# privefl/bigsnpr

Measured on AMD Instinct MI355X. Metric: SNP-cols/sec for bed_randomSVD k=20 (m*passes/wall), higher is better.
Workload: dtype i8 (2-bit codes x 24-bit (early block steps) / 16-bit (late block steps) fixed-point image of the fp64 basis in int8 slices, exact int32 MFMA accumulation; fp64 panel algebra and Rayleigh-Ritz)

## Files before the change

bigsnpr_amd/csrc/api.hip:

```cpp
#include <cxxabi.h>

#include <algorithm>
#include <cmath>
#include <cstring>
#include <limits>
#include <memory>

#include "bsn_internal.hpp"

namespace bsn {

static std::vector<int32_t> to_i32(const int64_t *ind, int64_t len, int64_t limit, const char *what) {
  std::vector<int32_t> v((size_t)len);
  if (!ind) {
    if (len > limit)
      fail("Tested %lld < %lld. Subscript out of bounds (%s).", (long long)(len - 1), (long long)limit, what);
    for (int64_t i = 0; i < len; i++) v[(size_t)i] = (int32_t)i;
    return v;
  }
  for (int64_t i = 0; i < len; i++) {
    if (ind[i] < 0 || ind[i] >= limit)
      fail("Tested %lld < %lld. Subscript out of bounds (%s).", (long long)ind[i], (long long)limit,
           what);
    v[(size_t)i] = (int32_t)ind[i];
// ... 318 lines not shown
  const double deno = deno_x * deno_y - num * num;
  res[j + (int64_t)k * m] = (deno == 0 || nona < 2) ? __longlong_as_double(0x7ff8000000000000LL)
                                                    : num * sqrt((nona - 2) / deno);
}
#pragma clang fp contract(on)

}

using namespace bsn;

extern "C" {

int bsn_selftest(void) {
  return guarded([&] {
    require_gpu();
    selftest();
  });
}

int bsn_op_last_kernel(bsn_op *op, char *buf, int64_t len) {
  return guarded([&] {
    if (!buf || len < 1) fail("bsn_op_last_kernel: no buffer");
    buf[0] = 0;
    if (!op->last_kernel) return;
    const char *mangled = hipKernelNameRefByPtr(op->last_kernel, op->bed->stream);
    if (!mangled) return;
    int status = 1;
    char *dem = abi::__cxa_demangle(mangled, nullptr, nullptr, &status);
    std::string name = (status == 0 && dem) ? dem : mangled;
    free(dem);
    const size_t par = name.find('(');
    if (par != std::string::npos) name.resize(par);
    snprintf(buf, (size_t)len, "%s", name.c_str());
  });
}

int bsn_op_create(bsn_bed *bed, const int64_t *ind_row, int64_t n, const int64_t *ind_col,
                  int64_t m, const double *center, const double *scale, bsn_op **out) {
  return guarded([&] {
    std::unique_ptr<bsn_op> op(new bsn_op());
    fill_op(op.get(), bed, ind_row, n, ind_col, m, center, scale);
    *out = op.release();
  });
}

int bsn_op_destroy(bsn_op *op) {
  return guarded([&] {
    if (op) {
      (void)hipSetDevice(op->bed->device);
      delete op;
    }
  });
}

int bsn_op_set_slices(bsn_op *op, int slices) {
  return guarded([&] {
    if (slices < 1 || slices > 7) fail("slices must be in 1..7");
    op->slices = slices;
  });
}

int bsn_op_prod(bsn_op *op, const double *d_X, int64_t ldx, int nvec, double *d_Y, int64_t ldy) {
  return guarded([&] {
    BSN_HIP(hipSetDevice(op->bed->device));
    op_prod(op, d_X, ldx, nvec, d_Y, ldy);
  });
// ... 455 lines not shown
```

bigsnpr_amd/csrc/bsn_internal.hpp:

```cpp
#pragma once
#include <hip/hip_runtime.h>
#include <stdint.h>

#include <atomic>
#include <cstdarg>
#include <cstdio>
#include <functional>
#include <cstdlib>
#include <memory>
#include <stdexcept>
#include <string>
#include <vector>

#include "bigsnpr_hip.h"

namespace bsn {
inline const char *abl_getenv(const char *name) {
#ifdef BSN_ABLATION
  return getenv(name);
#else
  (void)name;
  return nullptr;
#endif
}
// ... 319 lines not shown
void slab_upload_range(bsn_bed *b, int64_t j0, int64_t cnt);
struct SlabPart {
  bsn_bed *img;
  const std::vector<int64_t> &P;
  const std::vector<int64_t> &local;
  int64_t count() const { return (int64_t)P.size(); }
  const double *gather(const double *src, std::vector<double> &buf) const;
  void place(void *out, const void *part, size_t col_bytes) const;
};
void slab_walk(bsn_bed *bed, const int64_t *ind_col, int64_t m, const std::function<void(const SlabPart &)> &f);

hipEvent_t comm_time_begin(bsn_comm *c, hipStream_t st);
void comm_time_end(bsn_comm *c, hipEvent_t begin, int cls, hipStream_t st);
void comm_time_collect(bsn_comm *c, double ms[kCommClasses], int count[kCommClasses]);
bool comm_abort(bsn_comm *c);
void comm_allreduce_sum(bsn_comm *c, double *d_buf, int64_t count, hipStream_t st);
void comm_reduce_scatter_sum(bsn_comm *c, const double *d_send, double *d_recv, int64_t recv_count,
                             hipStream_t st);
void comm_all_gather(bsn_comm *c, const double *d_send, double *d_recv, int64_t send_count, hipStream_t st);

void op_poll_stats(bsn_op *op);
void op_na_blocks(bsn_op *op, int digit_cols);
void op_prod(bsn_op *op, const double *d_X, int64_t ldx, int nvec, double *d_Y, int64_t ldy);
void op_prod_acc(bsn_op *op, const double *d_X, int64_t ldx, int nvec, double *d_Y, int64_t ldy, double beta);
struct ProdSegment {
  int bs = 0, off = 0;
  const int32_t *d_rows = nullptr;
  double *d_out = nullptr;
};
bool op_prod_segments(bsn_op *op, const double *d_X, int64_t ldx, int nvec, int pieces, int stride, int nseg,
                      const ProdSegment *segs, const std::function<void(int)> &after);
void op_cprod(bsn_op *op, const double *d_X, int64_t ldx, int nvec, double *d_Z, int64_t ldz);
void op_cprod_prequant(bsn_op *op, const double *d_X, int64_t ldx, int nvec);
void op_cprod_raw(bsn_op *op, const double *d_X, int64_t ldx, int nvec, double *d_P, double *d_Q,
                  int64_t ld);
void require_bits(const bsn_bed *b, int bits, const char *what);
void op_row_sums_sq(bsn_op *op, double *d_out);
void op_row_counts(bsn_op *op, double *d_out);
void counts_weighted(bsn_op *op, const double *d_w, int64_t n_sub, int32_t *d_counts);
void counts_grouped(bsn_op *op, const int32_t *d_rows, const int32_t *d_group, int64_t n, int32_t G, const int32_t *d_gsize,
                    bool one_digit, int32_t *d_table, double ms_out[3]);
void group_counts_device(bsn_bed *bed, const int64_t *ind_row, int64_t n, const int32_t *group, int32_t G,
                         const int64_t *ind_col, int64_t m, DevBuf<int32_t> &d_table, double ms_out[3]);
void selftest();
void roctx_push(const char *name);
void roctx_pop();
struct RoctxRange {
  explicit RoctxRange(const char *name) { roctx_push(name); }
  ~RoctxRange() { roctx_pop(); }
  RoctxRange(const RoctxRange &) = delete;
  RoctxRange &operator=(const RoctxRange &) = delete;
};
void require_resident(const bsn_bed *b, const char *what);
void prof_begin(bsn_op *op, int kind, bool more = false);
void prof_end(bsn_op *op);
void prof_collect(bsn_op *op, double ms[kProfKinds], int count[kProfKinds]);

}
```

bigsnpr_amd/csrc/matvec.hip:

```cpp
#include <cmath>
#include <cstdlib>

#include "bsn_internal.hpp"
#include "byte_plan.hpp"
#include "prod_plan.hpp"
#include "prodt_sparse.hpp"
#include <type_traits>

namespace bsn {

typedef int v4i __attribute__((ext_vector_type(4)));
typedef int v8i __attribute__((ext_vector_type(8)));

static thread_local const void *g_last_kernel = nullptr;
#define BSN_KLAUNCH(kern, ...)                 \
  do {                                         \
    g_last_kernel = (const void *)(kern);      \
    hipLaunchKernelGGL(kern, __VA_ARGS__);     \
  } while (0)

__device__ __forceinline__ uint32_t lut4(uint32_t lut, uint32_t sel) {
  return __builtin_amdgcn_perm(lut, lut, sel);
}
__device__ __forceinline__ uint32_t perm8(uint32_t hi, uint32_t lo, uint32_t sel) {
  return __builtin_amdgcn_perm(hi, lo, sel);
}

constexpr uint32_t kLutG0 = 0x00020100u;
constexpr uint32_t kLutNA = 0x01000000u;
constexpr uint32_t kLutHom2 = 0x00010000u;
constexpr uint32_t kLutHet = 0x00000100u;
constexpr uint32_t kLutRaw = 0xFFFFFFFFu;

struct VecMeta {
// ... 166 lines not shown
        }
      }
    }
    for (int p = 0; p < nplanes; p++)
#pragma unroll
      for (int s = 0; s < S; s++) {
        const int col = v * S + s;
        int8_t *dst = q + ((kb * nplanes + p) * ncol + col) * 16;
        *(uint4 *)dst = p == 0 ? uint4{pk[0][s][0], pk[0][s][1], pk[0][s][2], pk[0][s][3]}
                               : uint4{pk[1][s][0], pk[1][s][1], pk[1][s][2], pk[1][s][3]};
      }
  }
  for (int off = 32; off > 0; off >>= 1) {
    shi += __shfl_down(shi, off); slo += __shfl_down(slo, off);
    shi2 += __shfl_down(shi2, off); slo2 += __shfl_down(slo2, off);
  }
  if (tid == 0) {
    atomicAdd((unsigned long long *)&meta[v].sum_hi, (unsigned long long)shi);
    atomicAdd((unsigned long long *)&meta[v].sum_lo, (unsigned long long)slo);
    if (mode >= 1) {
      atomicAdd((unsigned long long *)&meta[v].sum2_hi, (unsigned long long)shi2);
      atomicAdd((unsigned long long *)&meta[v].sum2_lo, (unsigned long long)slo2);
    }
  }
}

template <int NB, int NPLANE, int KC, bool RAW0, bool STATS, bool CONTIG, int TILES = 2, int WAVES = 8, int MINW = 1,
          int TAG = 0, bool TILED = false, int SGB = 0, bool NASKIP = false>
__global__ __launch_bounds__(64 * WAVES, MINW) void k_cprod(const uint8_t *__restrict__ img, int64_t pitch,
                                               const int32_t *__restrict__ cols, int64_t col0,
                                               int64_t m, const int8_t *__restrict__ xq,
                                               int32_t *__restrict__ acc_out, int64_t m_out,
                                               uint32_t lutA, uint32_t lutB, uint32_t lutC,
                                               int32_t *__restrict__ counts, int32_t n_pad_samples) {
  constexpr int NCOL = 16 * NB;
  constexpr int LD = KC / 256;
  constexpr int XS = KC / 16 * NCOL;
  __shared__ uint4 xs[2][XS];
  const int tid = threadIdx.x, wave = tid >> 6, lane = tid & 63;
  const int c = lane & 15, g = lane >> 4;
  constexpr int NT = 64 * WAVES;
  const int64_t wg_base = (int64_t)blockIdx.x * (WAVES * 16 * TILES);
  const int64_t snp_base = wg_base + wave * (16 * TILES);
  const uint8_t *rowp[TILES];
  uint32_t voff[TILES];
#pragma unroll
  for (int t = 0; t < TILES; t++) {
    int64_t j = snp_base + t * 16 + c;
    if (j > m - 1) j = m - 1;
    int64_t col = CONTIG ? col0 + j : (int64_t)cols[j];
    rowp[t] = img + col * pitch + g * 16;
    voff[t] = TILED ? (uint32_t)((((j - wg_base) >> 6) * (pitch >> 8)) * 16384 + (j & 63) * 256 + g * 16)
                    : (uint32_t)((j - wg_base) * pitch + g * 16);
  }
  static_assert(!TILED || (CONTIG && (WAVES * 16 * TILES) % 64 == 0), "streaming layout: whole 64-variant blocks");
  const __amdgpu_buffer_rsrc_t rs = __builtin_amdgcn_make_buffer_rsrc(
      (void *)(TILED ? img + (((col0 + wg_base) >> 6) * (pitch >> 8)) * 16384
                     : img + (col0 + (CONTIG ? wg_base : 0)) * pitch),
      0, 0x7fffffff, 0x00020000);
  typedef unsigned int v4u __attribute__((ext_vector_type(4)));
  auto gload = [&](const int t, const int off) -> uint4 {
    if constexpr (CONTIG) {
      const int soff = TILED ? ((off >> 8) << 14) + (off & 255) : off;
      const v4u r = __builtin_amdgcn_raw_buffer_load_b128(rs, (int)voff[t], soff, 0);
      return uint4{r.x, r.y, r.z, r.w};
    } else {
      return *(const uint4 *)(rowp[t] + off);
    }
  };
  const int nchunks = (int)(pitch * 4 / KC);
  const uint4 *xq4 = (const uint4 *)xq;

  v4i acc[TILES][NPLANE][NB];
#pragma unroll
  for (int t = 0; t < TILES; t++)
#pragma unroll
    for (int p = 0; p < NPLANE; p++)
#pragma unroll
      for (int nb = 0; nb < NB; nb++) acc[t][p][nb] = v4i{0, 0, 0, 0};
  uint32_t st_lo[TILES], st_hi[TILES], st_na[TILES];
#pragma unroll
  for (int t = 0; t < TILES; t++) st_lo[t] = st_hi[t] = st_na[t] = 0;

  constexpr int NX = (XS + NT - 1) / NT;
  static_assert(NX <= 4, "staging registers");
  constexpr bool XFULL = (XS % NT == 0);
  uint4 ga[2][TILES][LD];
  uint4 xr0 = {0, 0, 0, 0}, xr1 = {0, 0, 0, 0}, xr2 = {0, 0, 0, 0}, xr3 = {0, 0, 0, 0};
#pragma unroll
  for (int t = 0; t < TILES; t++)
#pragma unroll
    for (int it = 0; it < LD; it++) ga[0][t][it] = gload(t, it * 64);
  auto staged = [&](const int x) -> bool { return XFULL || tid + x * NT < XS; };
  if (staged(0)) xs[0][tid] = xq4[tid];
  if constexpr (NX > 1) if (staged(1)) xs[0][tid + NT] = xq4[tid + NT];
  if constexpr (NX > 2) if (staged(2)) xs[0][tid + 2 * NT] = xq4[tid + 2 * NT];
  if constexpr (NX > 3) if (staged(3)) xs[0][tid + 3 * NT] = xq4[tid + 3 * NT];
#pragma unroll
  for (int t = 0; t < TILES; t++)
#pragma unroll
    for (int it = 0; it < LD; it++)
      ga[1][t][it] = gload(t, (nchunks > 1 ? KC / 4 : 0) + it * 64);
  __syncthreads();

  auto chunk = [&](auto SETC, const int ch) {
    constexpr int SET = decltype(SETC)::value;
    const int ch1 = ch + 1 < nchunks ? ch + 1 : nchunks - 1;
    const int ch2 = ch + 2 < nchunks ? ch + 2 : nchunks - 1;
    {
      const uint4 *src = xq4 + (int64_t)ch1 * XS;
      auto at = [&](const int x) -> int { return XFULL ? tid + x * NT : (tid + x * NT < XS ? tid + x * NT : XS - 1); };
      xr0 = src[at(0)];
      if constexpr (NX > 1) xr1 = src[at(1)];
      if constexpr (NX > 2) xr2 = src[at(2)];
      if constexpr (NX > 3) xr3 = src[at(3)];
    }
    __builtin_amdgcn_sched_barrier(0);
    if constexpr (SGB & 2) __builtin_amdgcn_s_setprio(2);
    const int off2 = ch2 * (KC / 4);
    auto kstep = [&](const int t, const uint32_t w, const uint4 (&bv)[NB]) {
      uint32_t s0 = w & 0x03030303u, s1 = (w >> 2) & 0x03030303u,
               s2 = (w >> 4) & 0x03030303u, s3 = (w >> 6) & 0x03030303u;
      if constexpr (STATS) {
        const uint32_t lo = w & 0x55555555u;
        st_lo[t] += __popc(lo);
        st_hi[t] += __popc(w);
        st_na[t] += __popc(lo & (w >> 1));
      }
      static_assert(!NASKIP || (RAW0 && NPLANE == 2 && !STATS), "the skip is for the missing-value plane of the plain pass");
      bool plane1 = true;
      if constexpr (NASKIP) plane1 = __builtin_amdgcn_ballot_w64(((w & (w >> 1)) & 0x55555555u) != 0u) != 0ull;
#pragma unroll
      for (int p = 0; p < NPLANE; p++) {
        if (NASKIP && p == 1 && !plane1) continue;
        const uint32_t lut = p == 0 ? lutA : p == 1 ? lutB : lutC;
        v4i a;
        if (RAW0 && p == 0) {
          a = v4i{(int)s0, (int)s1, (int)s2, (int)s3};
        } else {
          a = v4i{(int)lut4(lut, s0), (int)lut4(lut, s1), (int)lut4(lut, s2), (int)lut4(lut, s3)};
        }
// ... 43 lines not shown
      constexpr int MSTEP = TILES * NPLANE * NB;
      __builtin_amdgcn_sched_group_barrier(0x100, NB, 0);
      __builtin_amdgcn_sched_group_barrier(0x002, 7, 0);
      auto slot = [&](auto IC) {
        constexpr int i = decltype(IC)::value;
        constexpr int nv = VSTEP * (i + 1) / MSTEP - VSTEP * i / MSTEP;
        __builtin_amdgcn_sched_group_barrier(0x008, 1, 0);
        if constexpr (nv > 0) __builtin_amdgcn_sched_group_barrier(0x002, nv, 0);
      };
      auto slots = [&](auto self, auto IC) {
        constexpr int i = decltype(IC)::value;
        if constexpr (i < MSTEP) {
          slot(IC);
          self(self, std::integral_constant<int, i + 1>{});
        }
      };
#pragma unroll
      for (int stp = 0; stp < LD * 4; stp++) {
        __builtin_amdgcn_sched_group_barrier(0x100, NB, 0);
        slots(slots, std::integral_constant<int, 0>{});
      }
      __builtin_amdgcn_sched_group_barrier(0x020, TILES * LD, 0);
    }
    __builtin_amdgcn_sched_barrier(0);
    if constexpr (SGB & 2) __builtin_amdgcn_s_setprio(0);
    {
      if (staged(0)) xs[SET ^ 1][tid] = xr0;
      if constexpr (NX > 1) if (staged(1)) xs[SET ^ 1][tid + NT] = xr1;
      if constexpr (NX > 2) if (staged(2)) xs[SET ^ 1][tid + 2 * NT] = xr2;
      if constexpr (NX > 3) if (staged(3)) xs[SET ^ 1][tid + 3 * NT] = xr3;
    }
    __syncthreads();
  };
  for (int ch = 0; ch < nchunks; ch += 2) {
    chunk(std::integral_constant<int, 0>{}, ch);
    if (ch + 1 < nchunks) chunk(std::integral_constant<int, 1>{}, ch + 1);
  }

#pragma unroll
  for (int t = 0; t < TILES; t++)
#pragma unroll
    for (int r = 0; r < 4; r++) {
      int64_t j = snp_base + t * 16 + g * 4 + r;
      if (j < m) {
#pragma unroll
        for (int p = 0; p < NPLANE; p++)
#pragma unroll
          for (int nb = 0; nb < NB; nb++)
            acc_out[((int64_t)p * m_out + j) * NCOL + nb * 16 + c] = acc[t][p][nb][r];
      }
    }
  if constexpr (STATS) {
#pragma unroll
    for (int t = 0; t < TILES; t++) {
      uint32_t lo = st_lo[t], hi = st_hi[t] - st_lo[t], na = st_na[t];
      lo += __shfl_xor(lo, 16); hi += __shfl_xor(hi, 16); na += __shfl_xor(na, 16);
      lo += __shfl_xor(lo, 32); hi += __shfl_xor(hi, 32); na += __shfl_xor(na, 32);
      const int64_t j = snp_base + t * 16 + c;
      if (g == 0 && j < m) {
        const int32_t n1 = (int32_t)(lo - na), n2 = (int32_t)(hi - na);
        *(int4 *)(counts + 4 * j) =
            int4{(int32_t)(pitch * 4) - n1 - n2 - (int32_t)na - n_pad_samples, n1, n2, (int32_t)na};
      }
    }
  }
}

__device__ __forceinline__ double horner(const int32_t *a, int S) {
  double r = 0;
  for (int s = S - 1; s >= 0; s--) r = r * 256.0 + (double)a[s];
  return r;
}
__device__ __forceinline__ double horner_sub(const int32_t *a, const int32_t *q, int k, int S) {
  double r = 0;
  for (int s = S - 1; s >= 0; s--) r = r * 256.0 + (double)((long long)a[s] - (long long)k * q[s]);
  return r;
}

template <int NCOL>
__global__ __launch_bounds__(128) void k_cprod_final(const int32_t *__restrict__ acc, int64_t m, int S, int nv,
                                                     const VecMeta *__restrict__ meta,
                                                     const double *__restrict__ center,
                                                     const double *__restrict__ scale, double *Z, int64_t ldz,
                                                     int has_q) {
  constexpr int ROW = 2 * NCOL + 1;
  __shared__ int32_t srow[128 * ROW];
  const int64_t j = (int64_t)blockIdx.x * 128 + threadIdx.x;
  if (j >= m) return;
  int32_t *my = srow + threadIdx.x * ROW;
  {
    const int4 *pa = (const int4 *)(acc + j * NCOL), *pq = (const int4 *)(acc + (m + j) * NCOL);
#pragma unroll
    for (int t = 0; t < NCOL / 4; t++) {
      const int4 x = pa[t];
      my[4 * t] = x.x; my[4 * t + 1] = x.y; my[4 * t + 2] = x.z; my[4 * t + 3] = x.w;
    }
    if (has_q) {
#pragma unroll
      for (int t = 0; t < NCOL / 4; t++) {
        const int4 x = pq[t];
        my[NCOL + 4 * t] = x.x; my[NCOL + 4 * t + 1] = x.y; my[NCOL + 4 * t + 2] = x.z; my[NCOL + 4 * t + 3] = x.w;
      }
    }
  }
  const double c = center ? center[j] : 0.0, s = scale ? scale[j] : 1.0;
  for (int v = 0; v < nv; v++) {
    const double P = has_q ? horner_sub(my + v * S, my + NCOL + v * S, 3, S) : horner(my + v * S, S);
    const double Q = has_q ? horner(my + NCOL + v * S, S) : 0.0;
    const double Sx = (double)meta[v].sum_hi * 16777216.0 + (double)meta[v].sum_lo;
    const double qs = meta[v].qscale;
    double z = qs > 0 ? (P - c * (Sx - Q)) / (s * qs) : 0.0 / s;
    if (P == 0.0 && Sx - Q == 0.0 && qs > 0) z = 0.0;
    if (meta[v].nonfinite) z = __longlong_as_double(0x7ff8000000000000LL);
    Z[j + v * ldz] = z;
  }
}

template <int NB, bool CONTIG, bool RAWP, bool HASQ = true, int TAG = 0, bool TILED = false>
__global__ __launch_bounds__(256) void k_prod(const uint8_t *__restrict__ img, int64_t pitch,
                                              const int32_t *__restrict__ cols, int64_t col0,
                                              int64_t m_pad, int64_t mc,
                                              const int8_t *__restrict__ wq,
                                              int32_t *__restrict__ acc_out, int64_t n_pad,
// ... 695 lines not shown
#pragma clang fp contract(on)

__global__ __launch_bounds__(256) void k_stats_summary(const int32_t *counts, int64_t m, int64_t n, int32_t *na,
                                                       unsigned long long *out) {
  long long s = 0, bad = 0;
  for (int64_t j = (int64_t)blockIdx.x * 256 + threadIdx.x; j < m; j += (int64_t)gridDim.x * 256) {
    const int4 c = *(const int4 *)(counts + 4 * j);
    s += c.w;
    na[j] = c.w;
    if (2 * ((int64_t)c.x + c.y + c.z) < n) bad++;
  }
  for (int off = 32; off > 0; off >>= 1) {
    s += __shfl_down(s, off);
    bad += __shfl_down(bad, off);
  }
  __shared__ long long sw[4], sb[4];
  if ((threadIdx.x & 63) == 0) {
    sw[threadIdx.x >> 6] = s;
    sb[threadIdx.x >> 6] = bad;
  }
  __syncthreads();
  if (threadIdx.x == 0) {
    s = sw[0] + sw[1] + sw[2] + sw[3];
    bad = sb[0] + sb[1] + sb[2] + sb[3];
    if (s) atomicAdd(&out[0], (unsigned long long)s);
    if (bad) atomicAdd(&out[1], (unsigned long long)bad);
  }
}

static bool use_tiled(const bsn_op *op) {
  return op->bed->d_tiled != nullptr && op->cols_contig && (op->col0 & 63) == 0;
}

template <int NPLANE, bool RAW0, bool STATS>
static void launch_cprod(bsn_op *op, int NB, const int8_t *q, int32_t *acc, uint32_t l0,
                         uint32_t l1, uint32_t l2, int32_t *counts = nullptr) {
  bsn_bed *b = op->bed;
  constexpr int KC = 512, TT = STATS ? 2 : 4;
  constexpr bool PLAIN = NPLANE == 2 && RAW0 && !STATS;
  if (b->pitch * 4 > 4000000) fail("more than 4e6 samples are not supported by the crossproduct kernel");
  const int32_t *cols = op->cols_contig ? nullptr : op->d_cols.p;
  const int32_t npad = (int32_t)(b->pitch * 4 - b->n);
  CprodFacts f;
  f.NB = NB, f.plain = PLAIN, f.stats = STATS, f.cols_contig = op->cols_contig, f.tiled = use_tiled(op);
  f.warm = op->prof_kind_override == 3, f.na_skip = op->na_skip_c;
  const CprodKernel k = choose_cprod(f);
  const uint8_t *image = k.tiled ? b->d_tiled : b->d_img;
  const int per_wg = 16 * k.tiles * k.waves;
  const dim3 grid((unsigned)((op->m + per_wg - 1) / per_wg)), block(64 * k.waves);
#define BSN_CPROD(NBV, CONTIGV, TV, WV, TAGV, TILEDV, SGBV, NASKIPV)                                                   \
  if (k == CprodKernel{NBV, CONTIGV, TV, WV, TAGV, TILEDV, SGBV, NASKIPV}) {                                           \
    BSN_KLAUNCH((k_cprod<NBV, NPLANE, KC, RAW0, STATS, CONTIGV, TV, WV, 1, TAGV, TILEDV, SGBV, NASKIPV>), grid, block, \
                0, b->stream, image, b->pitch, cols, op->col0, op->m, q, acc, op->m, l0, l1, l2, counts, npad);        \
    BSN_HIP(hipGetLastError());                                                                                        \
    return;                                                                                                            \
  }
  BSN_CPROD(1, false, 2, 8, 0, false, 0, false)
  BSN_CPROD(1, true, 2, 8, 0, false, 0, false)
  BSN_CPROD(1, true, 2, 8, 1, false, 0, false)
  BSN_CPROD(1, true, TT, 8, 0, true, 0, false)
  BSN_CPROD(1, true, TT, 8, 1, true, 0, false)
  BSN_CPROD(2, false, 2, 16, 0, false, 0, false)
  BSN_CPROD(2, true, 2, 16, 0, false, 3, false)
  BSN_CPROD(2, true, 2, 16, 0, true, 3, false)
  if constexpr (!STATS && NPLANE < 3) {
    BSN_CPROD(3, false, 2, 16, 0, false, 0, false)
    BSN_CPROD(3, true, 2, 16, 0, false, 3, false)
  }
  if constexpr (PLAIN) {
    BSN_CPROD(2, false, 2, 16, 0, false, 0, true)
    BSN_CPROD(2, true, 2, 16, 0, false, 0, true)
    BSN_CPROD(3, false, 2, 16, 0, false, 0, true)
    BSN_CPROD(3, true, 2, 16, 0, false, 0, true)
  }
#undef BSN_CPROD
  fail("internal: no crossproduct kernel with %d column blocks for this pass", NB);
}

static void launch_cprod_final(bsn_op *op, int NB, const int32_t *acc, int S, int nv, const VecMeta *meta, double *Z,
                               int64_t ldz, bool has_q) {
  auto go = [&](auto kern) {
    hipLaunchKernelGGL(kern, dim3((unsigned)((op->m + 127) / 128)), dim3(128), 0, op->bed->stream, acc, op->m, S, nv, meta,
                       op->d_center.p, op->d_scale.p, Z, ldz, has_q ? 1 : 0);
  };
  if (NB == 1) go(k_cprod_final<16>);
  else if (NB == 2) go(k_cprod_final<32>);
  else go(k_cprod_final<48>);
  BSN_HIP(hipGetLastError());
}

static void finish_fused_stats(bsn_op *op) {
  bsn_bed *b = op->bed;
  hipLaunchKernelGGL(k_binom_scale, dim3((unsigned)((op->m + 255) / 256)), dim3(256), 0, b->stream,
                     op->d_counts.p, op->m, op->d_center.p, op->d_scale.p);
  BSN_HIP(hipGetLastError());
  op->stats_pending = false;
  if (!op->h_na_total) BSN_HIP(hipHostMalloc((void **)&op->h_na_total, 2 * sizeof(long long), hipHostMallocDefault));
  op->h_na_total[0] = -1;
  op->h_na_total[1] = -1;
  unsigned long long *d_tot = (unsigned long long *)(op->d_counts.p + 4 * op->m);
  BSN_HIP(hipMemsetAsync(d_tot, 0, 16, b->stream));
  int gx = (int)((op->m + 1023) / 1024);
  if (gx > 1024) gx = 1024;
  hipLaunchKernelGGL(k_stats_summary, dim3(gx), dim3(256), 0, b->stream, op->d_counts.p, op->m, op->n,
                     op->d_na.ensure((size_t)op->m), d_tot);
  BSN_HIP(hipGetLastError());
  BSN_HIP(hipMemcpyAsync(op->h_na_total, d_tot, 16, hipMemcpyDeviceToHost, b->stream));
  op->na_poll = true;
}

void op_poll_stats(bsn_op *op) {
  if (!op->na_poll || !op->h_na_total) return;
  const long long t = *(volatile long long *)op->h_na_total;
  if (t < 0) return;
  op->na_poll = false;
  if (t == 0 && !getenv("BSN_FORCE_NA_PLANE")) op->no_na = true;
// ... 60 lines not shown
    BSN_HIP(hipMemsetAsync((uint8_t *)b->d_na_blocks + 4 * sizeof(long long), 1, 1, b->stream));
    BSN_HIP(hipMemcpyAsync(b->h_na_blocks, b->d_na_blocks, 4 * sizeof(long long), hipMemcpyDeviceToHost, b->stream));
    BSN_HIP(hipMemcpyAsync(b->h_na_blocks + 4, b->d_na_blocks + 4, sizeof(long long), hipMemcpyDeviceToHost, b->stream));
    b->na_blocks_state = 1;
    return;
  }
  if (b->na_blocks_state == 1) {
    if (*(volatile long long *)(b->h_na_blocks + 4) != 1) return;
    const long long *v = b->h_na_blocks;
    b->na_free[0] = v[1] > 0 ? (double)v[0] / (double)v[1] : 0.0;
    b->na_free[1] = v[3] > 0 ? (double)v[2] / (double)v[3] : 0.0;
    b->na_blocks_state = 2;
  }
  op->na_skip_c = b->na_free[0] >= min_free;
  op->na_skip_p = b->na_free[1] >= min_free;
}

static int cprod_vmax(const bsn_op *op, int S) { return cprod_vmax(op->bed->bits, op->stats_pending, S); }

void op_cprod_prequant(bsn_op *op, const double *d_X, int64_t ldx, int nvec) {
  bsn_bed *b = op->bed;
  const int S = op->slices;
  op->preq_X = nullptr;
  if (nvec <= 0 || nvec > cprod_vmax(op, S) || !op->rows_identity) return;
  const int64_t npad = n_padded(b);
  quantise(op, d_X, ldx, b->n, npad, nvec, 0, S, 16 * pick_nb(nvec * S), 1, 0, meta_buffer(op),
           op->d_q.ensure((size_t)npad * kMaxCols * 2));
  op->preq_X = d_X;
  op->preq_ldx = ldx;
  op->preq_nvec = nvec;
  op->preq_S = S;
}

void op_cprod(bsn_op *op, const double *d_X, int64_t ldx, int nvec, double *d_Z, int64_t ldz) {
  bsn_bed *b = op->bed;
  refuse_generic(b, "this function (it needs the streaming products)");
  const int S = op->slices;
  if (nvec <= 0) return;
  if (b->bits == 8 && byte_slices(b->pitch) > kByteMaxSlices)
    fail("the crossproduct on a dosage FBM supports at most %lld samples", (long long)(kByteMaxSlices * kSliceBytes));
  op_na_blocks(op, nvec * S);
  const bool have_digits = op->preq_X == d_X && op->preq_ldx == ldx && op->preq_nvec == nvec && d_X != nullptr &&
                           op->preq_S == S && nvec <= cprod_vmax(op, S);
  op->preq_X = nullptr;
  const double *xsrc = scatter_rows_if_needed(op, d_X, &ldx, nvec);
  const int64_t npad = n_padded(b);
  VecMeta *meta = meta_buffer(op);
  for (int v0 = 0, vmax = 0; v0 < nvec; v0 += vmax) {
    vmax = cprod_vmax(op, S);
    int nv = nvec - v0 < vmax ? nvec - v0 : vmax;
    int NB = pick_nb(nv * S), ncol = 16 * NB;
    int8_t *q = op->d_q.ensure((size_t)npad * kMaxCols * 2);
    const int nslice = b->bits == 8 ? byte_slices(b->pitch) : 1;
    int32_t *acc = op->d_acc.ensure(std::max((size_t)2 * op->m * kMaxCols, (size_t)nslice * 2 * op->m * ncol));
    if (!have_digits) quantise(op, xsrc + (int64_t)v0 * ldx, ldx, b->n, npad, nv, 0, S, ncol, 1, 0, meta, q);
    prof_begin(op, op->stats_pending ? 2 : NB == 3 ? 4 : 0);
    if (b->bits == 8) {
      const dim3 grid8((unsigned)((op->m + 127) / 128), (unsigned)nslice);
      const int32_t *cols8 = op->cols();
#define BSN_CPROD8(NBV, NAV, CV)                                                                          \
  BSN_KLAUNCH((k_cprod8<NBV, NAV, CV>), grid8, dim3(512), 0, b->stream, b->d_img, b->pitch, cols8, \
                     op->col0, op->m, q, acc, op->m, (int)(kSliceBytes / 256))
      if (NB == 1) {
        if (op->no_na) { if (op->cols_contig) BSN_CPROD8(1, false, true); else BSN_CPROD8(1, false, false); }
        else { if (op->cols_contig) BSN_CPROD8(1, true, true); else BSN_CPROD8(1, true, false); }
      } else {
        if (op->no_na) { if (op->cols_contig) BSN_CPROD8(2, false, true); else BSN_CPROD8(2, false, false); }
        else { if (op->cols_contig) BSN_CPROD8(2, true, true); else BSN_CPROD8(2, true, false); }
      }
#undef BSN_CPROD8
      BSN_HIP(hipGetLastError());
      prof_end(op);
      op->passes++;
      hipLaunchKernelGGL(k_cprod_final8, dim3((unsigned)((op->m + 255) / 256), nv), dim3(256), 0, b->stream, acc,
                         op->m, ncol, S, meta, op->d_center.p, op->d_scale.p, d_Z + (int64_t)v0 * ldz, ldz,
                         op->no_na ? 0 : 1, b->v_step, b->v_off, nslice);
      BSN_HIP(hipGetLastError());
      continue;
    }
    if (op->stats_pending) {
      if (!op->rows_identity) fail("internal: fused scaling statistics need all samples");
      launch_cprod<2, true, true>(op, NB, q, acc, kLutRaw, kLutNA, 0, op->d_counts.ensure((size_t)4 * op->m + 8));
    } else if (op->no_na) {
      launch_cprod<1, true, false>(op, NB, q, acc, kLutRaw, 0, 0);
    } else {
      launch_cprod<2, true, false>(op, NB, q, acc, kLutRaw, kLutNA, 0);
    }
    prof_end(op);
    op->passes++;
    if (op->late_center || op->late_scale) {
      hipStream_t up = upload_stream(b);
      if (op->late_center) copy_h2d(b, op->d_center.p, op->late_center, (size_t)op->m * 8, up);
      if (op->late_scale) copy_h2d(b, op->d_scale.p, op->late_scale, (size_t)op->m * 8, up);
      BSN_HIP(hipEventRecord(b->ev_up, up));
      BSN_HIP(hipStreamWaitEvent(b->stream, b->ev_up, 0));
      op->late_center = op->late_scale = nullptr;
    }
    const bool has_q = op->stats_pending || !op->no_na;
    if (op->stats_pending) finish_fused_stats(op);
    launch_cprod_final(op, NB, acc, S, nv, meta, d_Z + (int64_t)v0 * ldz, ldz, has_q);
  }
}

static void launch_prod(bsn_op *op, int NB, dim3 grid, int64_t m_pad, int64_t mc, const int8_t *q, int32_t *acc,
                        int64_t npad, uint32_t lutP, uint32_t lutQ, bool has_q) {
  bsn_bed *b = op->bed;
  const int32_t *cols = op->d_cols.p;
  const ProdKernel k = choose_prod(NB, op->cols_contig, use_tiled(op), lutP == kLutRaw, has_q, op->prof_kind_override == 3);
  const uint8_t *image = k.tiled ? b->d_tiled : b->d_img;
#define BSN_PROD(NBV, CV, RAWP, HASQ, TAGV, TILEDV)                                                                  \
  if (k == ProdKernel{NBV, CV, RAWP, HASQ, TAGV, TILEDV}) {                                                          \
    BSN_KLAUNCH((k_prod<NBV, CV, RAWP, HASQ, TAGV, TILEDV>), grid, dim3(256), 0, b->stream, image, b->pitch, cols,   \
                op->col0, m_pad, mc, q, acc, npad, lutP, lutQ);                                                      \
    BSN_HIP(hipGetLastError());                                                                                      \
    return;                                                                                                          \
  }
#define BSN_PROD6(NBV, CV, TILEDV)                                                                \
  BSN_PROD(NBV, CV, true, true, 0, TILEDV) BSN_PROD(NBV, CV, true, true, 1, TILEDV)               \
  BSN_PROD(NBV, CV, true, false, 0, TILEDV) BSN_PROD(NBV, CV, true, false, 1, TILEDV)             \
  BSN_PROD(NBV, CV, false, true, 0, TILEDV) BSN_PROD(NBV, CV, false, false, 0, TILEDV)
  BSN_PROD6(1, true, false) BSN_PROD6(1, true, true) BSN_PROD6(1, false, false)
  BSN_PROD6(2, true, false) BSN_PROD6(2, true, true) BSN_PROD6(2, false, false)
#undef BSN_PROD6
#undef BSN_PROD
  fail("internal: no product kernel with %d column blocks", NB);
}

static void launch_prodT(bsn_op *op, const ProdTKernel &k, const ProdTGrid &geo, dim3 seg_grid, const int8_t *q, int32_t *acc,
                         int64_t npad, uint32_t lutQ, int seg_bs, int seg_stride, int seg_off) {
  bsn_bed *b = op->bed;
  const dim3 grid = seg_bs > 0 ? seg_grid : dim3((unsigned)prodt_workgroups(geo));
#define BSN_PRODT(NBV, HASQV, TAGV, SGBV, NASKIPV, SPARSEV)                                                           \
  if (k == ProdTKernel{NBV, HASQV, TAGV, SGBV, NASKIPV, SPARSEV}) {                                                   \
    BSN_KLAUNCH((k_prodT<NBV, HASQV, 2, 16, TAGV, SGBV, NASKIPV, SPARSEV>), grid, dim3(1024), 0, b->stream, b->d_smaj, \
                b->rows_smaj, op->col0 / 512, geo, q, acc, npad, lutQ, seg_bs, seg_stride, seg_off);                  \
    BSN_HIP(hipGetLastError());                                                                                       \
    return;                                                                                                           \
  }
  BSN_PRODT(2, true, 0, 3, false, false) BSN_PRODT(2, true, 1, 3, false, false)
  BSN_PRODT(2, false, 0, 3, false, false) BSN_PRODT(2, false, 1, 3, false, false)
  BSN_PRODT(3, true, 0, 3, false, false) BSN_PRODT(3, false, 0, 3, false, false)
  BSN_PRODT(2, true, 0, 0, true, false) BSN_PRODT(3, true, 0, 0, true, false)
  BSN_PRODT(3, true, 0, 3, false, true) BSN_PRODT(3, true, 1, 3, false, true)
#undef BSN_PRODT
  fail("internal: no sample-major product kernel with %d column blocks", k.NB);
}

static void launch_prod_final(bsn_bed *b, int NB, const int32_t *acc, int64_t npad, int ky, int64_t rows_whole, int ky_whole, int S,
                              int nv, const VecMeta *meta,
                              const int32_t *d_rows, int64_t rows, double *Y, int64_t ldy, int sub_const, double beta,
                              int64_t blk_rows) {
  auto go = [&](auto kern) {
    hipLaunchKernelGGL(kern, dim3((unsigned)((rows + 255) / 256)), dim3(256), 0, b->stream, acc, npad, ky, rows_whole, ky_whole, S,
                       nv, meta, d_rows, rows, Y, ldy, sub_const, beta, blk_rows);
  };
  if (NB == 1) go(k_prod_final<16>);
  else if (NB == 2) go(k_prod_final<32>);
  else go(k_prod_final<48>);
  BSN_HIP(hipGetLastError());
}

static int device_cus() {
  static const int ncu = [] {
    hipDeviceProp_t pr;
    int dev = 0;
    return (hipGetDevice(&dev) == hipSuccess && hipGetDeviceProperties(&pr, dev) == hipSuccess && pr.multiProcessorCount > 0)
               ? pr.multiProcessorCount : 256;
  }();
  return ncu;
}

struct ProdSegments {
  int pieces, stride, nseg;
  const ProdSegment *segs;
  const std::function<void(int)> *after;
  bool done = false;
};
static void prod_planes(bsn_op *op, const double *d_X, const double *d_W2, int64_t ldx, int nvec,
                        double *d_Y, int64_t ldy, int mode, uint32_t lutP, uint32_t lutQ, int sub_const,
                        double beta, int S, ProdSegments *sg = nullptr) {
  bsn_bed *b = op->bed;
  refuse_generic(b, "this function (it needs the streaming products)");
  if (nvec <= 0) return;
  op->preq_X = nullptr;
  op_na_blocks(op, nvec * S);
  if (b->smaj_job) (void)image_smaj_poll(b);
  const bool has_q = lutQ != 0u && !(op->no_na && lutQ == kLutNA);
  ProdFacts f;
  f.bits = b->bits, f.n = b->n, f.m = op->m, f.pitch = b->pitch, f.col0 = op->col0, f.cols_contig = op->cols_contig;
  f.have_smaj = b->d_smaj != nullptr && !getenv("BSN_NO_SMAJ");
  f.mode = mode, f.raw_na = lutP == kLutRaw && lutQ == kLutNA, f.has_q = has_q;
  f.no_sparse = getenv("BSN_NO_SPARSE_PROD") != nullptr;
  f.nvec = nvec, f.S = S, f.segmented = sg != nullptr;
  if (f.have_smaj) f.ncu = device_cus();
  if (const char *e = getenv("BSN_PLAN_CUS")) f.ncu = std::max(1, atoi(e));
#ifdef BSN_ABLATION
  if (const char *e = getenv("BSN_KY")) f.ky = std::max(1, atoi(e));
  if (const char *e = getenv("BSN_KY_T")) f.ky_t = std::max(1, atoi(e));
  if (const char *e = getenv("BSN_KY_WHOLE")) f.ky_whole = std::max(1, atoi(e));
#endif
  const ProdPlan pl = plan_prod(f);
  if (pl.refuse == ProdRefusal::pitch_limit) fail("more than 6.7e7 samples are not supported by the product kernel");
// ... 328 lines not shown
```

bigsnpr_amd/csrc/prod_plan.hpp:

```cpp
#pragma once
#include <algorithm>
#include <cstdint>

#include "byte_plan.hpp"

#if defined(__HIPCC__)
#define BSN_PLAN_HD __host__ __device__ inline
#else
#define BSN_PLAN_HD inline
#endif

namespace bsn {
constexpr int kMaxCols = 48;
constexpr int kMetaVecs = 32;
inline int pick_nb(int ncols_needed) { return ncols_needed <= 16 ? 1 : ncols_needed <= 32 ? 2 : 3; }

inline int cprod_vmax(int bits, bool stats_pending, int S) {
  const int nbmax = (bits == 2 && !stats_pending) ? 3 : 2;
  int v = 16 * nbmax / S;
  if (v > kMetaVecs) v = kMetaVecs;
  return v < 1 ? 1 : v;
}

struct ProdFacts {
// ... 158 lines not shown
  return p;
}

struct CprodKernel {
  int NB;
  bool contig;
  int tiles, waves, tag;
  bool tiled;
  int sgb;
  bool naskip;
};
inline bool operator==(const CprodKernel &a, const CprodKernel &b) {
  return a.NB == b.NB && a.contig == b.contig && a.tiles == b.tiles && a.waves == b.waves && a.tag == b.tag &&
         a.tiled == b.tiled && a.sgb == b.sgb && a.naskip == b.naskip;
}
struct CprodFacts {
  int NB = 1;
  bool plain = true;
  bool stats = false;
  bool cols_contig = false;
  bool tiled = false;
  bool warm = false;
  bool na_skip = false;
};
inline CprodKernel choose_cprod(const CprodFacts &f) {
  if (f.plain && f.na_skip && f.NB >= 2) return {f.NB, f.cols_contig, 2, 16, 0, false, 0, true};
  if (f.NB == 3) return {3, f.cols_contig, 2, 16, 0, false, f.cols_contig ? 3 : 0, false};
  if (f.tiled) return f.NB == 1 ? CprodKernel{1, true, f.stats ? 2 : 4, 8, f.warm ? 1 : 0, true, 0, false}
                                : CprodKernel{2, true, 2, 16, 0, true, 3, false};
  if (f.NB == 1) return {1, f.cols_contig, 2, 8, f.cols_contig && f.warm ? 1 : 0, false, 0, false};
  return {2, f.cols_contig, 2, 16, 0, false, f.cols_contig ? 3 : 0, false};
}

struct ProdKernel {
  int NB;
  bool contig, rawp, hasq;
  int tag;
  bool tiled;
};
inline bool operator==(const ProdKernel &a, const ProdKernel &b) {
  return a.NB == b.NB && a.contig == b.contig && a.rawp == b.rawp && a.hasq == b.hasq && a.tag == b.tag && a.tiled == b.tiled;
}
inline ProdKernel choose_prod(int NB, bool cols_contig, bool tiled, bool rawp, bool has_q, bool warm) {
  return {NB, cols_contig, rawp, has_q, rawp && warm ? 1 : 0, cols_contig && tiled};
}

struct ProdTKernel {
  int NB;
  bool hasq;
  int tag, sgb;
  bool naskip, sparse;
};
inline bool operator==(const ProdTKernel &a, const ProdTKernel &b) {
  return a.NB == b.NB && a.hasq == b.hasq && a.tag == b.tag && a.sgb == b.sgb && a.naskip == b.naskip && a.sparse == b.sparse;
}
inline ProdTKernel choose_prodT(int NB, bool has_q, bool warm, bool na_skip, bool sparse_ok) {
  if (has_q && sparse_ok && NB == 3 && !na_skip) return {3, true, warm ? 1 : 0, 3, false, true};
  if (has_q && na_skip) return {NB, true, 0, 0, true, false};
  return {NB, has_q, NB == 2 && warm ? 1 : 0, 3, false, false};
}

}
```

Baseline: 39.26 million.

## Split tail workgroups of k_cprod over chunk slabs to fill the last wave

Plans the k_cprod grid so that whole waves of workgroups (CUs times resident blocks) run over all sample chunks as before. The leftover tail blocks are split along the chunk (sample) dimension into several slabs that write int32 partial sums to a scratch buffer. The final kernel then sums these partials for tail SNPs, and it now walks blocks in reverse order. The aim is to remove the under-filled last wave of the transpose product, at the cost of extra partial-sum traffic, an occupancy query, and a host-side planning pass before each launch.

```diff
diff --git a/bigsnpr_amd/csrc/api.hip b/bigsnpr_amd/csrc/api.hip
--- a/bigsnpr_amd/csrc/api.hip
+++ b/bigsnpr_amd/csrc/api.hip
@@ -374,6 +374,13 @@
     const size_t par = name.find('(');
     if (par != std::string::npos) name.resize(par);
     snprintf(buf, (size_t)len, "%s", name.c_str());
+  });
+}
+
+int bsn_op_cprod_grid(bsn_op *op, int nvec, int64_t *out9) {
+  return guarded([&] {
+    if (!out9) fail("bsn_op_cprod_grid: no buffer");
+    op_cprod_grid(op, nvec, out9);
   });
 }
 
diff --git a/bigsnpr_amd/csrc/bsn_internal.hpp b/bigsnpr_amd/csrc/bsn_internal.hpp
--- a/bigsnpr_amd/csrc/bsn_internal.hpp
+++ b/bigsnpr_amd/csrc/bsn_internal.hpp
@@ -375,6 +375,7 @@
                       const ProdSegment *segs, const std::function<void(int)> &after);
 void op_cprod(bsn_op *op, const double *d_X, int64_t ldx, int nvec, double *d_Z, int64_t ldz);
 void op_cprod_prequant(bsn_op *op, const double *d_X, int64_t ldx, int nvec);
+void op_cprod_grid(bsn_op *op, int nvec, int64_t *out);
 void op_cprod_raw(bsn_op *op, const double *d_X, int64_t ldx, int nvec, double *d_P, double *d_Q,
                   int64_t ld);
 void require_bits(const bsn_bed *b, int bits, const char *what);
diff --git a/bigsnpr_amd/csrc/matvec.hip b/bigsnpr_amd/csrc/matvec.hip
--- a/bigsnpr_amd/csrc/matvec.hip
+++ b/bigsnpr_amd/csrc/matvec.hip
@@ -1,5 +1,7 @@
 #include <cmath>
 #include <cstdlib>
+#include <map>
+#include <mutex>
 
 #include "bsn_internal.hpp"
 #include "byte_plan.hpp"
@@ -232,7 +234,8 @@
                                                int64_t m, const int8_t *__restrict__ xq,
                                                int32_t *__restrict__ acc_out, int64_t m_out,
                                                uint32_t lutA, uint32_t lutB, uint32_t lutC,
-                                               int32_t *__restrict__ counts, int32_t n_pad_samples) {
+                                               int32_t *__restrict__ counts, int32_t n_pad_samples,
+                                               const CprodGrid geo, int32_t *__restrict__ part_out) {
   constexpr int NCOL = 16 * NB;
   constexpr int LD = KC / 256;
   constexpr int XS = KC / 16 * NCOL;
@@ -240,7 +243,17 @@
   const int tid = threadIdx.x, wave = tid >> 6, lane = tid & 63;
   const int c = lane & 15, g = lane >> 4;
   constexpr int NT = 64 * WAVES;
-  const int64_t wg_base = (int64_t)blockIdx.x * (WAVES * 16 * TILES);
+  const int nchunks = (int)(pitch * 4 / KC);
+  constexpr bool GEO = CONTIG && !TILED && !STATS && NPLANE < 3 && KC == 512;
+  CprodSlab sl{(int)blockIdx.x, 0, 0, nchunks};
+  if constexpr (GEO) {
+    sl = cprod_slab(geo, blockIdx.x);
+    sl.block = __builtin_amdgcn_readfirstlane(sl.block), sl.slab = __builtin_amdgcn_readfirstlane(sl.slab);
+    sl.ch_begin = __builtin_amdgcn_readfirstlane(sl.ch_begin), sl.ch_end = __builtin_amdgcn_readfirstlane(sl.ch_end);
+  }
+  const int ch_begin = sl.ch_begin, ch_end = sl.ch_end;
+  if (ch_begin >= ch_end) return;
+  const int64_t wg_base = (int64_t)sl.block * (WAVES * 16 * TILES);
   const int64_t snp_base = wg_base + wave * (16 * TILES);
   const uint8_t *rowp[TILES];
   uint32_t voff[TILES];
@@ -268,7 +281,6 @@
       return *(const uint4 *)(rowp[t] + off);
     }
   };
-  const int nchunks = (int)(pitch * 4 / KC);
   const uint4 *xq4 = (const uint4 *)xq;
 
   v4i acc[TILES][NPLANE][NB];
@@ -290,23 +302,26 @@
 #pragma unroll
   for (int t = 0; t < TILES; t++)
 #pragma unroll
-    for (int it = 0; it < LD; it++) ga[0][t][it] = gload(t, it * 64);
+    for (int it = 0; it < LD; it++) ga[0][t][it] = gload(t, ch_begin * (KC / 4) + it * 64);
   auto staged = [&](const int x) -> bool { return XFULL || tid + x * NT < XS; };
-  if (staged(0)) xs[0][tid] = xq4[tid];
-  if constexpr (NX > 1) if (staged(1)) xs[0][tid + NT] = xq4[tid + NT];
-  if constexpr (NX > 2) if (staged(2)) xs[0][tid + 2 * NT] = xq4[tid + 2 * NT];
-  if constexpr (NX > 3) if (staged(3)) xs[0][tid + 3 * NT] = xq4[tid + 3 * NT];
+  {
+    const uint4 *src = xq4 + (int64_t)ch_begin * XS;
+    if (staged(0)) xs[0][tid] = src[tid];
+    if constexpr (NX > 1) if (staged(1)) xs[0][tid + NT] = src[tid + NT];
+    if constexpr (NX > 2) if (staged(2)) xs[0][tid + 2 * NT] = src[tid + 2 * NT];
+    if constexpr (NX > 3) if (staged(3)) xs[0][tid + 3 * NT] = src[tid + 3 * NT];
+  }
 #pragma unroll
   for (int t = 0; t < TILES; t++)
 #pragma unroll
     for (int it = 0; it < LD; it++)
-      ga[1][t][it] = gload(t, (nchunks > 1 ? KC / 4 : 0) + it * 64);
+      ga[1][t][it] = gload(t, (ch_end - ch_begin > 1 ? ch_begin + 1 : ch_begin) * (KC / 4) + it * 64);
   __syncthreads();
 
   auto chunk = [&](auto SETC, const int ch) {
     constexpr int SET = decltype(SETC)::value;
-    const int ch1 = ch + 1 < nchunks ? ch + 1 : nchunks - 1;
-    const int ch2 = ch + 2 < nchunks ? ch + 2 : nchunks - 1;
+    const int ch1 = ch + 1 < ch_end ? ch + 1 : ch_end - 1;
+    const int ch2 = ch + 2 < ch_end ? ch + 2 : ch_end - 1;
     {
       const uint4 *src = xq4 + (int64_t)ch1 * XS;
       auto at = [&](const int x) -> int { return XFULL ? tid + x * NT : (tid + x * NT < XS ? tid + x * NT : XS - 1); };
@@ -416,11 +431,19 @@
     }
     __syncthreads();
   };
-  for (int ch = 0; ch < nchunks; ch += 2) {
+  for (int ch = ch_begin; ch < ch_end; ch += 2) {
     chunk(std::integral_constant<int, 0>{}, ch);
-    if (ch + 1 < nchunks) chunk(std::integral_constant<int, 1>{}, ch + 1);
-  }
-
+    if (ch + 1 < ch_end) chunk(std::integral_constant<int, 1>{}, ch + 1);
+  }
+
+  int32_t *out = acc_out;
+  int64_t out_m = m_out, out_j0 = 0;
+  if constexpr (GEO) {
+    if (sl.block >= geo.blocks_whole) {
+      out_m = geo.m_rem, out_j0 = m - geo.m_rem;
+      out = part_out + (int64_t)sl.slab * NPLANE * out_m * NCOL;
+    }
+  }
 #pragma unroll
   for (int t = 0; t < TILES; t++)
 #pragma unroll
@@ -431,7 +454,7 @@
         for (int p = 0; p < NPLANE; p++)
 #pragma unroll
           for (int nb = 0; nb < NB; nb++)
-            acc_out[((int64_t)p * m_out + j) * NCOL + nb * 16 + c] = acc[t][p][nb][r];
+            out[((int64_t)p * out_m + j - out_j0) * NCOL + nb * 16 + c] = acc[t][p][nb][r];
       }
     }
   if constexpr (STATS) {
@@ -466,13 +489,31 @@
                                                      const VecMeta *__restrict__ meta,
                                                      const double *__restrict__ center,
                                                      const double *__restrict__ scale, double *Z, int64_t ldz,
-                                                     int has_q) {
+                                                     int has_q, const int32_t *__restrict__ part, int64_t m_rem,
+                                                     int slabs) {
   constexpr int ROW = 2 * NCOL + 1;
   __shared__ int32_t srow[128 * ROW];
-  const int64_t j = (int64_t)blockIdx.x * 128 + threadIdx.x;
+  const int64_t j = (int64_t)(gridDim.x - 1 - blockIdx.x) * 128 + threadIdx.x;
   if (j >= m) return;
   int32_t *my = srow + threadIdx.x * ROW;
-  {
+  if (slabs > 0 && j >= m - m_rem) {
+    const int nplane = has_q ? 2 : 1;
+    for (int p = 0; p < nplane; p++) {
+      long long d[NCOL];
+#pragma unroll
+      for (int c = 0; c < NCOL; c++) d[c] = 0;
+      const int4 *row = (const int4 *)(part + ((int64_t)p * m_rem + (j - (m - m_rem))) * NCOL);
+      for (int k = 0; k < slabs; k++, row += (int64_t)nplane * m_rem * (NCOL / 4)) {
+#pragma unroll
+        for (int t = 0; t < NCOL / 4; t++) {
+          const int4 v = row[t];
+          d[4 * t] += v.x, d[4 * t + 1] += v.y, d[4 * t + 2] += v.z, d[4 * t + 3] += v.w;
+        }
+      }
+#pragma unroll
+      for (int c = 0; c < NCOL; c++) my[p * NCOL + c] = (int32_t)d[c];
+    }
+  } else {
     const int4 *pa = (const int4 *)(acc + j * NCOL), *pq = (const int4 *)(acc + (m + j) * NCOL);
 #pragma unroll
     for (int t = 0; t < NCOL / 4; t++) {
@@ -1234,9 +1275,44 @@
   return op->bed->d_tiled != nullptr && op->cols_contig && (op->col0 & 63) == 0;
 }
 
+static int device_cus() {
+  static const int ncu = [] {
+    hipDeviceProp_t pr;
+    int dev = 0;
+    return (hipGetDevice(&dev) == hipSuccess && hipGetDeviceProperties(&pr, dev) == hipSuccess && pr.multiProcessorCount > 0)
+               ? pr.multiProcessorCount : 256;
+  }();
+  return ncu;
+}
+
+static thread_local CprodGridFacts g_cprod_facts;
+static CprodGrid cprod_geometry(bsn_op *op, const void *kern, int per_wg, int threads, int NB, int nplane) {
+  static std::mutex mu;
+  static std::map<const void *, int> held;
+  int resident;
+  {
+    std::lock_guard<std::mutex> lk(mu);
+    auto it = held.find(kern);
+    if (it == held.end()) {
+      int nb = 0;
+      if (hipOccupancyMaxActiveBlocksPerMultiprocessor(&nb, kern, threads, 0) != hipSuccess || nb < 1) nb = 1;
+      it = held.emplace(kern, nb).first;
+    }
+    resident = it->second;
+  }
+  CprodGridFacts f;
+  f.m = op->m, f.per_wg = per_wg, f.nchunks = (int)(op->bed->pitch * 4 / 512), f.pitch = op->bed->pitch;
+  f.NB = NB, f.nplane = nplane, f.ncu = device_cus(), f.resident = resident;
+  if (const char *e = getenv("BSN_PLAN_CUS")) f.ncu = std::max(1, atoi(e));
+  if (const char *e = getenv("BSN_CPROD_SLABS")) f.slabs = std::max(1, atoi(e));
+  g_cprod_facts = f;
+  return plan_cprod(f);
+}
+
 template <int NPLANE, bool RAW0, bool STATS>
 static void launch_cprod(bsn_op *op, int NB, const int8_t *q, int32_t *acc, uint32_t l0,
-                         uint32_t l1, uint32_t l2, int32_t *counts = nullptr) {
+                         uint32_t l1, uint32_t l2, int32_t *counts = nullptr, CprodGrid *geo = nullptr,
+                         int32_t *part = nullptr) {
   bsn_bed *b = op->bed;
   constexpr int KC = 512, TT = STATS ? 2 : 4;
   constexpr bool PLAIN = NPLANE == 2 && RAW0 && !STATS;
@@ -1249,11 +1325,25 @@
   const CprodKernel k = choose_cprod(f);
   const uint8_t *image = k.tiled ? b->d_tiled : b->d_img;
   const int per_wg = 16 * k.tiles * k.waves;
-  const dim3 grid((unsigned)((op->m + per_wg - 1) / per_wg)), block(64 * k.waves);
+  const bool geo_ok = geo && k.contig && !k.tiled && !STATS && NPLANE < 3 && !getenv("BSN_CPROD_ONE_SPLIT");
+  CprodGrid one;
+  one.blocks = one.blocks_whole = (int)((op->m + per_wg - 1) / per_wg), one.nchunks = (int)(b->pitch * 4 / KC);
+  const bool planning = geo && !acc;
+  if (planning && !geo_ok) {
+    *geo = one;
+    return;
+  }
+  const CprodGrid g = geo && !planning ? *geo : one;
+  const dim3 grid((unsigned)cprod_workgroups(g)), block(64 * k.waves);
 #define BSN_CPROD(NBV, CONTIGV, TV, WV, TAGV, TILEDV, SGBV, NASKIPV)                                                   \
   if (k == CprodKernel{NBV, CONTIGV, TV, WV, TAGV, TILEDV, SGBV, NASKIPV}) {                                           \
-    BSN_KLAUNCH((k_cprod<NBV, NPLANE, KC, RAW0, STATS, CONTIGV, TV, WV, 1, TAGV, TILEDV, SGBV, NASKIPV>), grid, block, \
-                0, b->stream, image, b->pitch, cols, op->col0, op->m, q, acc, op->m, l0, l1, l2, counts, npad);        \
+    auto kern = k_cprod<NBV, NPLANE, KC, RAW0, STATS, CONTIGV, TV, WV, 1, TAGV, TILEDV, SGBV, NASKIPV>;                \
+    if (planning) {                                                                                                    \
+      *geo = cprod_geometry(op, (const void *)kern, per_wg, 64 * k.waves, NB, NPLANE);                                 \
+      return;                                                                                                          \
+    }                                                                                                                  \
+    BSN_KLAUNCH(kern, grid, block, 0, b->stream, image, b->pitch, cols, op->col0, op->m, q, acc, op->m, l0, l1, l2,    \
+                counts, npad, g, part);                                                                                \
     BSN_HIP(hipGetLastError());                                                                                        \
     return;                                                                                                            \
   }
@@ -1280,10 +1370,10 @@
 }
 
 static void launch_cprod_final(bsn_op *op, int NB, const int32_t *acc, int S, int nv, const VecMeta *meta, double *Z,
-                               int64_t ldz, bool has_q) {
+                               int64_t ldz, bool has_q, const CprodGrid &geo, const int32_t *part) {
   auto go = [&](auto kern) {
     hipLaunchKernelGGL(kern, dim3((unsigned)((op->m + 127) / 128)), dim3(128), 0, op->bed->stream, acc, op->m, S, nv, meta,
-                       op->d_center.p, op->d_scale.p, Z, ldz, has_q ? 1 : 0);
+                       op->d_center.p, op->d_scale.p, Z, ldz, has_q ? 1 : 0, part, geo.m_rem, geo.slabs);
   };
   if (NB == 1) go(k_cprod_final<16>);
   else if (NB == 2) go(k_cprod_final<32>);
@@ -1410,6 +1500,29 @@
   op->preq_S = S;
 }
 
+static void cprod_on_image(bsn_op *op, int NB, const int8_t *q, int32_t *acc, CprodGrid *geo, int32_t *part) {
+  if (op->stats_pending) {
+    if (!op->rows_identity) fail("internal: fused scaling statistics need all samples");
+    launch_cprod<2, true, true>(op, NB, q, acc, kLutRaw, kLutNA, 0, op->d_counts.ensure((size_t)4 * op->m + 8), geo, part);
+  } else if (op->no_na) {
+    launch_cprod<1, true, false>(op, NB, q, acc, kLutRaw, 0, 0, nullptr, geo, part);
+  } else {
+    launch_cprod<2, true, false>(op, NB, q, acc, kLutRaw, kLutNA, 0, nullptr, geo, part);
+  }
+}
+
+void op_cprod_grid(bsn_op *op, int nvec, int64_t *out) {
+  require_bits(op->bed, 2, "the grid of k_cprod");
+  if (nvec <= 0) fail("op_cprod_grid: no vectors");
+  CprodGrid g;
+  g_cprod_facts = CprodGridFacts();
+  g_cprod_facts.per_wg = g_cprod_facts.ncu = g_cprod_facts.resident = 0;
+  const int S = op->slices;
+  op_na_blocks(op, nvec * S);
+  cprod_on_image(op, pick_nb(std::min(nvec, cprod_vmax(op, S)) * S), nullptr, nullptr, &g, nullptr);
+  out[0] = g.blocks, out[1] = g.blocks_whole, out[2] = g.slabs, out[3] = g.cps, out[4] = g.nchunks, out[5] = g.m_rem;
+  out[6] = g_cprod_facts.per_wg, out[7] = g_cprod_facts.ncu, out[8] = g_cprod_facts.resident;
+}
 void op_cprod(bsn_op *op, const double *d_X, int64_t ldx, int nvec, double *d_Z, int64_t ldz) {
   bsn_bed *b = op->bed;
   refuse_generic(b, "this function (it needs the streaming products)");
@@ -1430,7 +1543,12 @@
     int NB = pick_nb(nv * S), ncol = 16 * NB;
     int8_t *q = op->d_q.ensure((size_t)npad * kMaxCols * 2);
     const int nslice = b->bits == 8 ? byte_slices(b->pitch) : 1;
-    int32_t *acc = op->d_acc.ensure(std::max((size_t)2 * op->m * kMaxCols, (size_t)nslice * 2 * op->m * ncol));
+    CprodGrid geo;
+    if (b->bits == 2) cprod_on_image(op, NB, q, nullptr, &geo, nullptr);
+    const size_t acc_words = std::max((size_t)2 * op->m * kMaxCols, (size_t)nslice * 2 * op->m * ncol);
+    const size_t part_words = (size_t)cprod_partial_words(geo, op->stats_pending || !op->no_na ? 2 : 1, NB);
+    int32_t *acc = op->d_acc.ensure(acc_words + part_words);
+    int32_t *part = acc + acc_words;
     if (!have_digits) quantise(op, xsrc + (int64_t)v0 * ldx, ldx, b->n, npad, nv, 0, S, ncol, 1, 0, meta, q);
     prof_begin(op, op->stats_pending ? 2 : NB == 3 ? 4 : 0);
     if (b->bits == 8) {
@@ -1456,14 +1574,7 @@
       BSN_HIP(hipGetLastError());
       continue;
     }
-    if (op->stats_pending) {
-      if (!op->rows_identity) fail("internal: fused scaling statistics need all samples");
-      launch_cprod<2, true, true>(op, NB, q, acc, kLutRaw, kLutNA, 0, op->d_counts.ensure((size_t)4 * op->m + 8));
-    } else if (op->no_na) {
-      launch_cprod<1, true, false>(op, NB, q, acc, kLutRaw, 0, 0);
-    } else {
-      launch_cprod<2, true, false>(op, NB, q, acc, kLutRaw, kLutNA, 0);
-    }
+    cprod_on_image(op, NB, q, acc, &geo, part);
     prof_end(op);
     op->passes++;
     if (op->late_center || op->late_scale) {
@@ -1476,7 +1587,7 @@
     }
     const bool has_q = op->stats_pending || !op->no_na;
     if (op->stats_pending) finish_fused_stats(op);
-    launch_cprod_final(op, NB, acc, S, nv, meta, d_Z + (int64_t)v0 * ldz, ldz, has_q);
+    launch_cprod_final(op, NB, acc, S, nv, meta, d_Z + (int64_t)v0 * ldz, ldz, has_q, geo, part);
   }
 }
 
@@ -1536,16 +1647,6 @@
   else if (NB == 2) go(k_prod_final<32>);
   else go(k_prod_final<48>);
   BSN_HIP(hipGetLastError());
-}
-
-static int device_cus() {
-  static const int ncu = [] {
-    hipDeviceProp_t pr;
-    int dev = 0;
-    return (hipGetDevice(&dev) == hipSuccess && hipGetDeviceProperties(&pr, dev) == hipSuccess && pr.multiProcessorCount > 0)
-               ? pr.multiProcessorCount : 256;
-  }();
-  return ncu;
 }
 
 struct ProdSegments {
diff --git a/bigsnpr_amd/csrc/prod_plan.hpp b/bigsnpr_amd/csrc/prod_plan.hpp
--- a/bigsnpr_amd/csrc/prod_plan.hpp
+++ b/bigsnpr_amd/csrc/prod_plan.hpp
@@ -214,6 +214,79 @@
   return {2, f.cols_contig, 2, 16, 0, false, f.cols_contig ? 3 : 0, false};
 }
 
+struct CprodGridFacts {
+  int64_t m = 0;
+  int per_wg = 512;
+  int nchunks = 1;
+  int64_t pitch = 128;
+  int NB = 1, nplane = 2;
+  int ncu = 256;
+  int resident = 1;
+  bool one_split = false;
+  int slabs = 0;
+};
+struct CprodGrid {
+  int blocks = 0, blocks_whole = 0;
+  int slabs = 0, cps = 0;
+  int nchunks = 0;
+  int64_t m_rem = 0;
+};
+struct CprodSlab {
+  int block, slab;
+  int ch_begin, ch_end;
+};
+constexpr int kCprodMaxSlabs = 24;
+BSN_PLAN_HD int64_t cprod_workgroups(const CprodGrid &g) {
+  return (int64_t)g.blocks_whole + (int64_t)(g.blocks - g.blocks_whole) * g.slabs;
+}
+inline int64_t cprod_partial_words(const CprodGrid &g, int nplane, int NB) {
+  return (int64_t)g.slabs * nplane * g.m_rem * 16 * NB;
+}
+BSN_PLAN_HD CprodSlab cprod_slab(const CprodGrid &g, uint32_t wg) {
+  CprodSlab s;
+  if (wg < (uint32_t)g.blocks_whole) {
+    s.block = (int)wg, s.slab = 0, s.ch_begin = 0, s.ch_end = g.nchunks;
+    return s;
+  }
+  const uint32_t r = wg - (uint32_t)g.blocks_whole, nrest = (uint32_t)(g.blocks - g.blocks_whole);
+  s.slab = (int)(r / nrest);
+  s.block = g.blocks_whole + (int)(r - (uint32_t)s.slab * nrest);
+  s.ch_begin = s.slab * g.cps;
+  s.ch_end = s.ch_begin + g.cps < g.nchunks ? s.ch_begin + g.cps : g.nchunks;
+  return s;
+}
+inline CprodGrid plan_cprod(const CprodGridFacts &f) {
+  CprodGrid g;
+  g.blocks = (int)((f.m + f.per_wg - 1) / f.per_wg);
+  g.nchunks = f.nchunks;
+  g.blocks_whole = g.blocks;
+  const int64_t slots = (int64_t)std::max(1, f.ncu) * std::max(1, f.resident);
+  const int64_t whole = g.blocks / slots * slots, rest = g.blocks - whole;
+  if (f.one_split || rest == 0 || f.nchunks <= 1) return g;
+  if (rest >= std::max(1, f.ncu) && f.slabs == 0) return g;
+  const double slab_cost = 1.0 * 2.0 * (double)f.nplane * 16.0 * f.NB * 4.0 / (double)f.pitch;
+  int best = 1;
+  double best_score = -1e300;
+  for (int c = 1; c <= kCprodMaxSlabs && c <= f.nchunks; c++) {
+    const int cps = (f.nchunks + c - 1) / c;
+    if ((f.nchunks + cps - 1) / cps != c) continue;
+    const int64_t W = rest * c;
+    const double fill = (double)W / ((double)slots * (double)((W + slots - 1) / slots));
+    const double score = fill - (c > 1 ? slab_cost * c : 0.0);
+    if (score > best_score + 1e-9) best_score = score, best = c;
+  }
+  if (f.slabs > 0) {
+    const int c = std::min(f.slabs, f.nchunks), cps = (f.nchunks + c - 1) / c;
+    best = (f.nchunks + cps - 1) / cps;
+  }
+  if (best == 1) return g;
+  g.blocks_whole = (int)whole;
+  g.cps = (f.nchunks + best - 1) / best;
+  g.slabs = best;
+  g.m_rem = f.m - whole * f.per_wg;
+  return g;
+}
+
 struct ProdKernel {
   int NB;
   bool contig, rawp, hasq;
```

After: 39.83 million, median of 6. 1.01x the previous value.
